# AI4Science-WestlakeU/safediffcon

Measured on AMD Instinct MI355X. Metric: sampled control trajectories/sec (1000-step DDPM), higher is better.
Workload: dtype f32; 1 GPU; C4: 2D smoke Unet3D_with_Conv3D dim=64 (1,2,4) state (B,32,7,64,64), B=64 per GPU, guided 1000-step DDPM, conformal quantile on; batch_per_gpu=64, global_batch=64, step=U-Net + guidance + posterior update of the whole batch, one hipGraph replay, parallelism=batch-sharded x1, no data-path collective, conv_precision=fp32

## Files before the change

### include/sdc.h

```cpp
#ifndef SDC_H
#define SDC_H

#include <stddef.h>
#include <stdint.h>

#ifdef __cplusplus
extern "C" {
#endif

#define SDC_OK 0
#define SDC_EINVAL (-1)
#define SDC_EALIGN (-2)
#define SDC_EHIP (-3)
#define SDC_ENULL (-4)

int sdc_version(void);
int sdc_last_error(char* buf, size_t cap);

typedef struct SdcConvDesc {
    int32_t B, Cin0, Cin1, Cout;
    int32_t iD, iH, iW;
    int32_t oD, oH, oW;
    int32_t kD, kH, kW;
    int32_t sD, sH, sW;
// ... 36 lines not shown

int sdc_chan_norm(const float* x, const float* g, const float* residual, float* y, int B, int C, int64_t S,
                  int mode, float eps, void* stream);

int sdc_linattn(const float* qkv, float* ctx, float* out, int outer, int inner, int heads, int64_t n,
                int64_t q_so, int64_t q_sc, int64_t q_si, int64_t o_so, int64_t o_sc, int64_t o_si, void* stream);

size_t sdc_linattn_block_bytes(int outer, int inner, int C, int64_t n);
int sdc_linattn_block(const float* x, const float* g_pre, const float* wqkv, const float* wo, const float* bo,
                      const float* g_post, float* work, float* y, int outer, int inner, int C, int64_t n,
                      int64_t so, int64_t sc, int64_t si, int pre_mode, int post_mode, float eps, void* stream);
int sdc_linattn_block_gn(const float* x_raw, const float* gn_stats, const float* gn_gamma, const float* gn_beta, int gn_G,
                         const float* gn_residual, const float* g_pre, const float* wqkv, const float* wo, const float* bo,
                         const float* g_post, float* work, float* y, int outer, int inner, int C, int64_t n,
                         int64_t so, int64_t sc, int64_t si, int pre_mode, int post_mode, float eps, void* stream);

size_t sdc_pack_linattn_f16_bytes(int C);
int sdc_pack_linattn_f16(const float* wqkv, const float* wo, int C, void* dst, void* stream);
size_t sdc_linattn_block_f16_bytes(int outer, int inner, int C, int64_t n);
int sdc_linattn_block_f16(const float* x, const float* g_pre, const float* wqkv, const float* wo, const void* wpk, const float* bo,
                          const float* g_post, void* work, float* y, int outer, int inner, int C, int64_t n,
                          int64_t so, int64_t sc, int64_t si, int pre_mode, int post_mode, float eps, void* stream);
int sdc_linattn_block_gn_f16(const float* x_raw, const float* gn_stats, const float* gn_gamma, const float* gn_beta, int gn_G,
                             const float* gn_residual, const float* g_pre, const float* wqkv, const float* wo, const void* wpk,
                             const float* bo, const float* g_post, void* work, float* y, int outer, int inner, int C, int64_t n,
                             int64_t so, int64_t sc, int64_t si, int pre_mode, int post_mode, float eps, void* stream);
int sdc_linattn_block_f16_ok(int C, int64_t n);

int sdc_tattn_block(const float* x, const float* g_pre, const float* wqkv, const float* wo, const float* rot,
                    const float* bias, float* y, int outer, int inner, int C, int ntok, int64_t so, int64_t sc,
// ... 238 lines not shown
```

### safediffcon_amd/_lib.py

```python
import ctypes as C
import os

_HERE = os.path.dirname(os.path.abspath(__file__))
LIB_PATH = os.path.join(_HERE, "libsdc_hip.so")

SDC_MODEL_BURGERS, SDC_MODEL_TOKAMAK, SDC_MODEL_SMOKE = 0, 1, 2

_f32p = C.c_void_p
_i32p = C.c_void_p
_stream = C.c_void_p
_i64 = C.c_int64


class SdcConvDesc(C.Structure):
    _fields_ = [(n, C.c_int32) for n in (
        "B", "Cin0", "Cin1", "Cout", "iD", "iH", "iW", "oD", "oH", "oW", "kD", "kH", "kW", "sD", "sH", "sW",
        "pD", "pH", "pW", "uD", "uH", "uW", "up_mode", "precision")] + [
        ("x0s", C.c_int64 * 5), ("x1s", C.c_int64 * 5), ("ys", C.c_int64 * 5), ("rs", C.c_int64 * 5)]


class SdcStepDesc(C.Structure):
    _fields_ = [(n, C.c_int32) for n in (
        "model", "B", "d0", "d1", "d2", "d3", "guide", "clip", "impose", "cond_idx", "pad_zero", "use_max",
        "has_wgt", "skip_draws", "ddim")] + [("_pad", C.c_int32), ("seed", C.c_uint64)]
# ... 49 lines not shown
    "sdc_gn_apply": (C.c_int, [_f32p, _f32p, _f32p, _f32p, _f32p, _i32p, _i64, _i64, _i64, _f32p, _f32p,
                               C.c_int, C.c_int, C.c_int, _i64, _stream]),
    "sdc_gn_fused_ok": (C.c_int, [C.c_int, C.c_int, C.c_int, _i64]),
    "sdc_gn_fused": (C.c_int, [_f32p, _f32p, _f32p, _f32p, _i32p, _i64, _i64, _i64, _f32p, _f32p, C.c_int, C.c_int, C.c_int, _i64,
                               C.c_float, _stream]),
    "sdc_gn_pointwise_out": (C.c_int, [_f32p, _f32p, _f32p, _f32p, _f32p, _f32p, _f32p, _f32p, C.c_int, C.c_int, C.c_int, C.c_int, _i64,
                                       _i64, _i64, _i64, _i64, _stream]),
    "sdc_chan_norm": (C.c_int, [_f32p, _f32p, _f32p, _f32p, C.c_int, C.c_int, _i64, C.c_int, C.c_float, _stream]),
    "sdc_linattn": (C.c_int, [_f32p, _f32p, _f32p, C.c_int, C.c_int, C.c_int, _i64, _i64, _i64, _i64, _i64, _i64,
                              _i64, _stream]),
    "sdc_linattn_block_bytes": (C.c_size_t, [C.c_int, C.c_int, C.c_int, _i64]),
    "sdc_linattn_block": (C.c_int, [_f32p, _f32p, _f32p, _f32p, _f32p, _f32p, _f32p, _f32p, C.c_int, C.c_int, C.c_int, _i64,
                                    _i64, _i64, _i64, C.c_int, C.c_int, C.c_float, _stream]),
    "sdc_linattn_block_gn": (C.c_int, [_f32p, _f32p, _f32p, _f32p, C.c_int, _f32p, _f32p, _f32p, _f32p, _f32p, _f32p, _f32p, _f32p,
                                       C.c_int, C.c_int, C.c_int, _i64, _i64, _i64, _i64, C.c_int, C.c_int, C.c_float, _stream]),
    "sdc_pack_linattn_f16_bytes": (C.c_size_t, [C.c_int]),
    "sdc_pack_linattn_f16": (C.c_int, [_f32p, _f32p, C.c_int, C.c_void_p, _stream]),
    "sdc_linattn_block_f16_bytes": (C.c_size_t, [C.c_int, C.c_int, C.c_int, _i64]),
    "sdc_linattn_block_f16": (C.c_int, [_f32p, _f32p, _f32p, _f32p, C.c_void_p, _f32p, _f32p, C.c_void_p, _f32p, C.c_int, C.c_int,
                                        C.c_int, _i64, _i64, _i64, _i64, C.c_int, C.c_int, C.c_float, _stream]),
    "sdc_linattn_block_gn_f16": (C.c_int, [_f32p, _f32p, _f32p, _f32p, C.c_int, _f32p, _f32p, _f32p, _f32p, C.c_void_p, _f32p, _f32p,
                                           C.c_void_p, _f32p, C.c_int, C.c_int, C.c_int, _i64, _i64, _i64, _i64, C.c_int, C.c_int,
                                           C.c_float, _stream]),
    "sdc_linattn_block_f16_ok": (C.c_int, [C.c_int, _i64]),
    "sdc_tattn_block": (C.c_int, [_f32p, _f32p, _f32p, _f32p, _f32p, _f32p, _f32p, C.c_int, C.c_int, C.c_int, C.c_int,
                                  _i64, _i64, _i64, C.c_float, _stream]),
    "sdc_pack_tattn_f16_bytes": (C.c_size_t, []),
    "sdc_pack_tattn_f16": (C.c_int, [_f32p, _f32p, C.c_void_p, _stream]),
    "sdc_tattn_block_f16": (C.c_int, [_f32p, _f32p, C.c_void_p, _f32p, _f32p, _f32p, C.c_int, C.c_int, C.c_int, C.c_int,
                                      _i64, _i64, _i64, C.c_float, _stream]),
# ... 124 lines not shown
```

### safediffcon_amd/build.py

```python
import os
import subprocess
import sys

HERE = os.path.dirname(os.path.abspath(__file__))
CSRC = os.path.join(HERE, "csrc")
LIB = os.path.join(HERE, "libsdc_hip.so")
SOURCES = ["sdc_api.hip", "sdc_conv.hip", "sdc_conv_wino.hip", "sdc_conv_f16.hip", "sdc_conv_stem_f16.hip", "sdc_conv_stem_x3.hip", "sdc_conv_gemm_x3.hip", "sdc_conv_wino_x3.hip", "sdc_norm.hip", "sdc_attn.hip", "sdc_lablock.hip", "sdc_lablock_f16.hip", "sdc_tablock.hip", "sdc_tablock_f16.hip", "sdc_tablock_x3.hip", "sdc_step.hip", "sdc_solver.hip", "sdc_grad.hip", "sdc_wgrad_f16.hip", "sdc_attn_bwd.hip", "sdc_kstar.hip", "sdc_smoke.hip", "sdc_linear.hip", "sdc_optim.hip"]
HEADERS = ["sdc_common.h", "sdc_lablock_tile.h", "sdc_conv.h", "sdc_conv_wino3s.inc", "sdc_conv_wino2s.inc", "sdc_conv_pw2.inc"]
HIPCC = os.environ.get("HIPCC", "/opt/rocm/bin/hipcc")
FLAGS = ["--offload-arch=gfx950", "-O3", "-fPIC", "-std=c++17", "-Wall", "-Wno-unused-function"]


def source_hash():
    import hashlib
    h = hashlib.sha256()
    for f in SOURCES + HEADERS:
        with open(os.path.join(CSRC, f), "rb") as fh:
            h.update(fh.read())
    with open(os.path.join(HERE, "..", "include", "sdc.h"), "rb") as fh:
        h.update(fh.read())
    return h.hexdigest()[:16]


def _stale(out, deps):
# ... 44 lines not shown
```

### safediffcon_amd/csrc/sdc_conv_stem_x3.hip

```cpp
#include "sdc_conv.h"

using namespace sdcconv;

namespace {

typedef __bf16 bf16x8 __attribute__((ext_vector_type(8)));

constexpr int SX_BM = 64, SX_BN = 256, SX_NT = 256;

struct StemX3Args {
    const float* x;
    const __bf16* wb;
    const float* bias;
    float* y;
    int64_t xs[5], ys[5];
    int B, Cin, Cout, oD, oH, W, lgW;
    int kD;
    int Hs, NR;
    int Ntot, ntiles, mtiles;
    int itemsB;
    int plane;
};

__device__ __forceinline__ void split3(float x, __bf16& h, __bf16& m, __bf16& l) {
#pragma clang fp contract(off)
    h = (__bf16)x;
    const float r = x - (float)h;
    m = (__bf16)r;
    l = (__bf16)(r - (float)m);
}

template <int KH, int ITB>
__global__ __launch_bounds__(SX_NT) __attribute__((amdgpu_waves_per_eu(1))) SDC_NO_DS_MERGE void conv_stem_x3_kernel(const StemX3Args a) {
    constexpr int TAPS = KH * 7;
    constexpr int NS = (TAPS + 1) / 2;
    constexpr int SS = KH == 7 ? 5 : NS;
    constexpr int NSUB = NS / SS;
    static_assert(NSUB * SS == NS, "whole sub-stages");
    constexpr int HH = KH - 1;
    constexpr int APC = SS * SX_BM * 32;
    constexpr int ASZ = 3 * APC;
    constexpr int NIA = 3 * SS * SX_BM * 2;
    constexpr int ITA = (NIA + SX_NT - 1) / SX_NT;
    extern __shared__ __attribute__((aligned(16))) char lds[];

// ... 267 lines not shown
```

### safediffcon_amd/csrc/sdc_conv_wino_x3.hip

```cpp
#include "sdc_conv.h"

using namespace sdcconv;

namespace {

typedef __bf16 bf16x8 __attribute__((ext_vector_type(8)));
typedef __bf16 bf16x4 __attribute__((ext_vector_type(4)));
typedef float w2f2 __attribute__((ext_vector_type(2)));
typedef float nfloat4 __attribute__((ext_vector_type(4)));
typedef float nfloat2 __attribute__((ext_vector_type(2)));

__device__ __forceinline__ w2f2 pk_add2(w2f2 a, w2f2 b) { w2f2 r; asm("v_pk_add_f32 %0, %1, %2" : "=v"(r) : "v"(a), "v"(b)); return r; }
__device__ __forceinline__ w2f2 pk_sub2(w2f2 a, w2f2 b) { w2f2 r; asm("v_pk_add_f32 %0, %1, %2 neg_lo:[0,1] neg_hi:[0,1]" : "=v"(r) : "v"(a), "v"(b)); return r; }
__device__ __forceinline__ w2f2 pk_fma2(w2f2 a, w2f2 b, w2f2 c) { w2f2 r; asm("v_pk_fma_f32 %0, %1, %2, %3" : "=v"(r) : "v"(a), "v"(b), "v"(c)); return r; }
__device__ __forceinline__ w2f2 pk_fms2(w2f2 a, w2f2 b, w2f2 c) { w2f2 r; asm("v_pk_fma_f32 %0, %1, %2, %3 neg_lo:[0,0,1] neg_hi:[0,0,1]" : "=v"(r) : "v"(a), "v"(b), "v"(c)); return r; }
__device__ __forceinline__ w2f2 pk_fnma2(w2f2 a, w2f2 b, w2f2 c) { w2f2 r; asm("v_pk_fma_f32 %0, %1, %2, %3 neg_lo:[0,1,0] neg_hi:[0,1,0]" : "=v"(r) : "v"(a), "v"(b), "v"(c)); return r; }
__device__ __forceinline__ w2f2 pk_sumdiff(w2f2 c) {
    w2f2 r;
    asm("v_pk_add_f32 %0, %1, %1 op_sel:[0,1] op_sel_hi:[1,0] neg_hi:[0,1]" : "=v"(r) : "v"(c));
    return r;
}
__device__ __forceinline__ w2f2 pk_sumdiff_fwd(w2f2 c) {
    w2f2 r;
    asm("v_pk_add_f32 %0, %1, %1 op_sel:[0,1] op_sel_hi:[0,1] neg_hi:[0,1]" : "=v"(r) : "v"(c));
// ... 22 lines not shown
#pragma unroll
    for (int i = 0; i < 2; ++i) u[i] = (b4 ? w[2 + i] : w[i]) + __shfl_xor(b4 ? w[i] : w[2 + i], 16, 64);
    double t = (b3 ? u[1] : u[0]) + __shfl_xor(b3 ? u[0] : u[1], 8, 64);
    t += __shfl_xor(t, 4, 64);
    t += __shfl_xor(t, 2, 64);
    t += __shfl_xor(t, 1, 64);
    return t;
}

__device__ __forceinline__ uint32_t cvt_pk_bf16(float a, float b) {
    typedef __bf16 bf16x2 __attribute__((ext_vector_type(2)));
    return __builtin_bit_cast(uint32_t, __builtin_convertvector(w2f2{a, b}, bf16x2));
}
__device__ __forceinline__ float bf16_lo(uint32_t p) { return __builtin_bit_cast(float, p << 16); }
__device__ __forceinline__ float bf16_hi(uint32_t p) { return __builtin_bit_cast(float, p & 0xFFFF0000u); }
__device__ __forceinline__ void split3(float x, __bf16& h, __bf16& m, __bf16& l) {
#pragma clang fp contract(off)
    h = (__bf16)x;
    const float r = x - (float)h;
    m = (__bf16)r;
    l = (__bf16)(r - (float)m);
}

constexpr int X3_BM = 64, X3_TILES = 64, X3_SK = 16;
constexpr int X3_PC = 4 * 64 * X3_SK * 2;
constexpr int X3_IMG = 3 * X3_PC;
constexpr int X3_U = 0, X3_V = 2 * X3_IMG;
constexpr int X3_SCR = 4 * X3_IMG;
constexpr int X3_STASH = X3_SCR + 4 * 8 * 8;
constexpr int X3_LDS = X3_STASH + 256 * 8 * 4;
constexpr int X3_RUN = 4 * 64 * X3_SK;

struct WinoX3Args {
    SdcConvDesc d;
    const float* x0;
    const float* x1;
    const __bf16* wb;
// ... 477 lines not shown
```

### safediffcon_amd/csrc/sdc_lablock.hip

```cpp
#include "sdc_common.h"
#include "sdc_lablock_tile.h"

namespace {

struct LaArgs {
    const float* x;
    const float* g_pre;
    const float* wqkv;
    const float* wo;
    const float* bo;
    const float* g_post;
    float* part;
    float* tt;
    float* y;
    const float* gn_stats; const float* gn_gamma; const float* gn_beta; const float* gn_res;
    float* gn_hout;
    int gn_G;
    int inner, nsplit, tiles_per_split, ntiles, tiles_per_blk;
    int pre_mode, post_mode;
    float eps;
    int64_t so, sc, si;
};

template <int C>
__device__ __forceinline__ void norm_tile(float (&v)[C / 4], const float* __restrict__ g, int mode, float eps,
                                          float* __restrict__ xs, float* __restrict__ xr, float* __restrict__ red, int tid) {
    constexpr int CG = C / 4;
    const int tok = tid & 63, grp = tid >> 6;
    if (xr) {
#pragma unroll
        for (int k = 0; k < CG; ++k) xr[(grp * CG + k) * XP + tok] = v[k];
    }
    typedef float la_f2 __attribute__((ext_vector_type(2)));
    la_f2 s2 = {0.f, 0.f};
    if (mode == 0) {
#pragma unroll
        for (int k = 0; k < CG; k += 2) s2 += la_f2{v[k], v[k + 1]};
// ... 355 lines not shown
}

}

extern "C" size_t sdc_linattn_block_bytes(int outer, int inner, int C, int64_t n) {
    if (outer <= 0 || inner <= 0 || n <= 0 || (C != 64 && C != 128)) return 0;
    const int64_t nseq = (int64_t)outer * inner;
    const int ns = pick_nsplit(nseq, (int)(n / TT));
    return sizeof(float) * (size_t)(nseq * ns * 4 * 32 * (C + 2) + nseq * HID * C);
}

namespace {
int linattn_block_impl(const float* x, const float* gn_stats, const float* gn_gamma, const float* gn_beta, int gn_G,
                       const float* gn_res, const float* g_pre, const float* wqkv, const float* wo, const float* bo,
                       const float* g_post, float* work, float* y, int outer, int inner, int C, int64_t n,
                       int64_t so, int64_t sc, int64_t si, int pre_mode, int post_mode, float eps, void* stream) {
    SDC_REQUIRE(x && g_pre && wqkv && wo && work && y, SDC_ENULL, "sdc_linattn_block: null pointer");
    SDC_REQUIRE(C == 64 || C == 128, SDC_EINVAL, "sdc_linattn_block: dim must be 64 or 128 (got %d)", C);
    SDC_REQUIRE(outer > 0 && inner > 0 && n > 0 && n % TT == 0, SDC_EINVAL, "sdc_linattn_block: tokens must be a multiple of 64");
    SDC_REQUIRE((pre_mode == 0 || pre_mode == 1) && post_mode >= -1 && post_mode <= 1, SDC_EINVAL, "sdc_linattn_block: bad norm mode");
    SDC_REQUIRE(post_mode < 0 || g_post, SDC_ENULL, "sdc_linattn_block: post norm needs its gain");
    const int64_t nseq = (int64_t)outer * inner;
    SDC_REQUIRE(nseq < 65536, SDC_EINVAL, "sdc_linattn_block: outer*inner must be < 65536");
    SDC_REQUIRE(sc > 0 && sc < (1ll << 27), SDC_EINVAL, "sdc_linattn_block: channel stride must stay below 2^27 elements (32-bit lane offsets)");
    LaArgs a;
    a.x = x; a.g_pre = g_pre; a.wqkv = wqkv; a.wo = wo; a.bo = bo; a.g_post = g_post; a.y = y;
    a.gn_stats = gn_stats; a.gn_gamma = gn_gamma; a.gn_beta = gn_beta; a.gn_res = gn_res; a.gn_G = gn_G; a.gn_hout = nullptr;
    a.inner = inner; a.ntiles = (int)(n / TT);
    a.nsplit = pick_nsplit(nseq, a.ntiles);
    a.tiles_per_split = (a.ntiles + a.nsplit - 1) / a.nsplit;
    a.nsplit = (a.ntiles + a.tiles_per_split - 1) / a.tiles_per_split;
    {
// ... 7 lines not shown
    a.so = so; a.sc = sc; a.si = si;
    hipStream_t s = sdc::as_stream(stream);
    const dim3 g1((unsigned)a.nsplit, (unsigned)nseq), gm(4, (unsigned)nseq),
        g2((unsigned)((a.ntiles + a.tiles_per_blk - 1) / a.tiles_per_blk), (unsigned)nseq);
    const size_t ldsb = sizeof(float) * (size_t)((C + HID) * XP + 8 * TT + 2 * C);
    const size_t ldsb2 = sizeof(float) * (size_t)((C + HID) * XP + 8 * TT + C * XP + 2 * C);
    static std::atomic<uint64_t> attr0{0}, attr1{0}, attr2{0};
    static std::atomic<uint64_t> attr3{0};
    SDC_LDS_OPTIN(attr0, (la_blk_ctx<128, false>), 96 * 1024, "sdc_linattn_block");
    SDC_LDS_OPTIN(attr1, la_blk_out<128>, 128 * 1024, "sdc_linattn_block");
    SDC_LDS_OPTIN(attr2, la_blk_out<64>, 96 * 1024, "sdc_linattn_block");
    SDC_LDS_OPTIN(attr3, (la_blk_ctx<128, true>), 96 * 1024, "sdc_linattn_block");
    const bool gn = gn_stats != nullptr;
    LaArgs a2 = a;
    if (gn) { a.gn_hout = y; a2.x = y; a2.gn_stats = nullptr; }
    if (C == 64) {
        if (gn) hipLaunchKernelGGL((la_blk_ctx<64, true>), g1, dim3(NT), ldsb, s, a);
        else hipLaunchKernelGGL((la_blk_ctx<64, false>), g1, dim3(NT), ldsb, s, a);
        hipLaunchKernelGGL(la_blk_mid<64>, gm, dim3(NT), 0, s, a);
        hipLaunchKernelGGL(la_blk_out<64>, g2, dim3(NT), ldsb2, s, a2);
    } else {
        if (gn) hipLaunchKernelGGL((la_blk_ctx<128, true>), g1, dim3(NT), ldsb, s, a);
        else hipLaunchKernelGGL((la_blk_ctx<128, false>), g1, dim3(NT), ldsb, s, a);
        hipLaunchKernelGGL(la_blk_mid<128>, gm, dim3(NT), 0, s, a);
        hipLaunchKernelGGL(la_blk_out<128>, g2, dim3(NT), ldsb2, s, a2);
    }
    return sdc::check_launch("sdc_linattn_block");
}
}

extern "C" int sdc_linattn_block(const float* x, const float* g_pre, const float* wqkv, const float* wo, const float* bo,
                                 const float* g_post, float* work, float* y, int outer, int inner, int C, int64_t n,
                                 int64_t so, int64_t sc, int64_t si, int pre_mode, int post_mode, float eps, void* stream) {
    return linattn_block_impl(x, nullptr, nullptr, nullptr, 0, nullptr, g_pre, wqkv, wo, bo, g_post, work, y, outer, inner, C, n, so, sc,
                              si, pre_mode, post_mode, eps, stream);
}

extern "C" int sdc_linattn_block_gn(const float* x_raw, const float* gn_stats, const float* gn_gamma, const float* gn_beta, int gn_G,
                                    const float* gn_residual, const float* g_pre, const float* wqkv, const float* wo, const float* bo,
                                    const float* g_post, float* work, float* y, int outer, int inner, int C, int64_t n,
                                    int64_t so, int64_t sc, int64_t si, int pre_mode, int post_mode, float eps, void* stream) {
    SDC_REQUIRE(gn_stats && gn_gamma && gn_beta, SDC_ENULL, "sdc_linattn_block_gn: null GroupNorm pointer");
    SDC_REQUIRE(gn_G > 0 && (C == 64 || C == 128) && C % gn_G == 0, SDC_EINVAL, "sdc_linattn_block_gn: groups must divide the channels");
    return linattn_block_impl(x_raw, gn_stats, gn_gamma, gn_beta, gn_G, gn_residual, g_pre, wqkv, wo, bo, g_post, work, y, outer, inner,
                              C, n, so, sc, si, pre_mode, post_mode, eps, stream);
}
```

### safediffcon_amd/csrc/sdc_lablock_tile.h

```cpp
#pragma once
#include "sdc_common.h"

namespace {

constexpr int NT = 256;
constexpr int TT = 64;
constexpr int XP = TT + 1;
constexpr int HID = 128;
constexpr float LOG2E = 1.4426950408889634f;
typedef float f32x16 __attribute__((ext_vector_type(16)));

typedef __attribute__((address_space(1))) float* la_gptr;
typedef __attribute__((address_space(1))) char* la_gcptr;
__device__ __forceinline__ la_gptr la_uni(const float* p) {
    const uint64_t u = reinterpret_cast<uint64_t>(p);
    const uint32_t lo = __builtin_amdgcn_readfirstlane((uint32_t)u), hi = __builtin_amdgcn_readfirstlane((uint32_t)(u >> 32));
    return (la_gptr)(((uint64_t)hi << 32) | lo);
}
__device__ __forceinline__ float la_ld(la_gptr base, uint32_t byte_off) { return *(la_gptr)((la_gcptr)base + byte_off); }
__device__ __forceinline__ void la_st(la_gptr base, uint32_t byte_off, float v) { *(la_gptr)((la_gcptr)base + byte_off) = v; }

__device__ __forceinline__ float la_max3(float a, float b, float c) { float r; asm("v_max3_f32 %0, %1, %2, %3" : "=v"(r) : "v"(a), "v"(b), "v"(c)); return r; }

template <int C>
// ... 60 lines not shown
```

### safediffcon_amd/csrc/sdc_tablock_x3.hip

```cpp
#include "sdc_common.h"

namespace {

constexpr int NT = 512;
constexpr int C = 64;
constexpr int NS = 8;
constexpr int XP = NS * 33;
constexpr int XF = 68;
constexpr int XPP = 32 * XF + 8;
constexpr int WQKV_E = 3 * 4 * 64 * 8;
constexpr int HEAD_E = WQKV_E + 2 * 2 * 64 * 8;
constexpr int WPK_E = 4 * 3 * HEAD_E;
constexpr int WBUF_B = 3 * HEAD_E * 2;
constexpr int REGB_B = NS * XPP * 4;
typedef float f32x16 __attribute__((ext_vector_type(16)));
typedef float nfloat4 __attribute__((ext_vector_type(4)));
typedef __bf16 bf16x8 __attribute__((ext_vector_type(8)));
typedef uint32_t u32x4 __attribute__((ext_vector_type(4)));
static_assert(WBUF_B <= REGB_B && 32 * XP * 4 <= REGB_B, "region B holds a head's weights and a y half");
static_assert(WBUF_B % (16 * NT) == 0, "whole 16-byte words per thread");

struct TaArgs {
    const float* x; const float* g; const __bf16* wpk; const float* rot; const float* bias;
    float* y;
// ... 8 lines not shown
typedef __attribute__((address_space(1))) float* gptr_t;
typedef __attribute__((address_space(1))) char* gcptr_t;
__device__ __forceinline__ gptr_t uni(const float* p) {
    const uint64_t u = reinterpret_cast<uint64_t>(p);
    const uint32_t lo = __builtin_amdgcn_readfirstlane((uint32_t)u), hi = __builtin_amdgcn_readfirstlane((uint32_t)(u >> 32));
    return (gptr_t)(((uint64_t)hi << 32) | lo);
}
__device__ __forceinline__ float ldu(gptr_t base, uint32_t byte_off) { return *(gptr_t)((gcptr_t)base + byte_off); }
__device__ __forceinline__ void stu(gptr_t base, uint32_t byte_off, float v) { *(gptr_t)((gcptr_t)base + byte_off) = v; }

typedef float ta2 __attribute__((ext_vector_type(2)));
__device__ __forceinline__ ta2 ta_rot(ta2 x, ta2 cs) {
#pragma clang fp contract(off)
    const float t0 = x.x * cs.x, t1 = x.y * cs.x;
    return ta2{__builtin_fmaf(-x.y, cs.y, t0), __builtin_fmaf(x.x, cs.y, t1)};
}

__device__ __forceinline__ void split3(float x, __bf16& h, __bf16& m, __bf16& l) {
#pragma clang fp contract(off)
    h = (__bf16)x;
    const float r = x - (float)h;
    m = (__bf16)r;
    l = (__bf16)(r - (float)m);
}

__global__ __launch_bounds__(NT) void ta_block_x3_kernel(const TaArgs a) {
    extern __shared__ __attribute__((aligned(16))) unsigned char smem_x3[];
    unsigned char* const wA = smem_x3;
    unsigned char* const rB = smem_x3 + WBUF_B;
    float* const xim = reinterpret_cast<float*>(rB);
    float* const ys = reinterpret_cast<float*>(rB);
    float* const biasT = reinterpret_cast<float*>(rB + REGB_B);
    float* const rotcs = biasT + 4 * 32 * 33;
    float* const red = rotcs + 2 * 32 * 16;

    const int tid = threadIdx.x, lane = tid & 63, wave = tid >> 6, l31 = lane & 31, lh = lane >> 5;
    const int nblk = a.nblk, nwg = gridDim.x, w = blockIdx.x;
    const bool xcd = ((nblk & 7) == 0) && ((nwg & 7) == 0);
// ... 258 lines not shown
```

Baseline: 0.3024 trajectories/s.

## Add bf16x3 split MFMA path for linear-attention block context and output kernels

Adds new context and output kernels for the linear-attention block. Activations and weights are split into three bf16 pieces so the projections run on bf16 MFMA while keeping accuracy close to fp32, and the default entry points now take this path for supported channel and token counts. The split3 helper moves into a shared header and the LaArgs struct is exposed so the new kernels can use it. The cost is the split work and larger LDS use per block, which may limit how many blocks fit on a CU.

Measured after the change: 0.3068 trajectories/s, median of 6. +1.5%, better.

```diff
diff --git a/include/sdc.h b/include/sdc.h
--- a/include/sdc.h
+++ b/include/sdc.h
@@ -74,6 +74,14 @@
                          const float* gn_residual, const float* g_pre, const float* wqkv, const float* wo, const float* bo,
                          const float* g_post, float* work, float* y, int outer, int inner, int C, int64_t n,
                          int64_t so, int64_t sc, int64_t si, int pre_mode, int post_mode, float eps, void* stream);
+int sdc_linattn_block_sel(const float* x, const float* g_pre, const float* wqkv, const float* wo, const float* bo,
+                          const float* g_post, float* work, float* y, int outer, int inner, int C, int64_t n,
+                          int64_t so, int64_t sc, int64_t si, int pre_mode, int post_mode, float eps, int impl, void* stream);
+int sdc_linattn_block_gn_sel(const float* x_raw, const float* gn_stats, const float* gn_gamma, const float* gn_beta, int gn_G,
+                             const float* gn_residual, const float* g_pre, const float* wqkv, const float* wo, const float* bo,
+                             const float* g_post, float* work, float* y, int outer, int inner, int C, int64_t n,
+                             int64_t so, int64_t sc, int64_t si, int pre_mode, int post_mode, float eps, int impl, void* stream);
+int sdc_linattn_block_x3_ok(int C, int64_t n);
 
 size_t sdc_pack_linattn_f16_bytes(int C);
 int sdc_pack_linattn_f16(const float* wqkv, const float* wo, int C, void* dst, void* stream);
diff --git a/safediffcon_amd/_lib.py b/safediffcon_amd/_lib.py
--- a/safediffcon_amd/_lib.py
+++ b/safediffcon_amd/_lib.py
@@ -87,6 +87,11 @@
                                     _i64, _i64, _i64, C.c_int, C.c_int, C.c_float, _stream]),
     "sdc_linattn_block_gn": (C.c_int, [_f32p, _f32p, _f32p, _f32p, C.c_int, _f32p, _f32p, _f32p, _f32p, _f32p, _f32p, _f32p, _f32p,
                                        C.c_int, C.c_int, C.c_int, _i64, _i64, _i64, _i64, C.c_int, C.c_int, C.c_float, _stream]),
+    "sdc_linattn_block_sel": (C.c_int, [_f32p, _f32p, _f32p, _f32p, _f32p, _f32p, _f32p, _f32p, C.c_int, C.c_int, C.c_int, _i64,
+                                        _i64, _i64, _i64, C.c_int, C.c_int, C.c_float, C.c_int, _stream]),
+    "sdc_linattn_block_gn_sel": (C.c_int, [_f32p, _f32p, _f32p, _f32p, C.c_int, _f32p, _f32p, _f32p, _f32p, _f32p, _f32p, _f32p, _f32p,
+                                           C.c_int, C.c_int, C.c_int, _i64, _i64, _i64, _i64, C.c_int, C.c_int, C.c_float, C.c_int, _stream]),
+    "sdc_linattn_block_x3_ok": (C.c_int, [C.c_int, _i64]),
     "sdc_pack_linattn_f16_bytes": (C.c_size_t, [C.c_int]),
     "sdc_pack_linattn_f16": (C.c_int, [_f32p, _f32p, C.c_int, C.c_void_p, _stream]),
     "sdc_linattn_block_f16_bytes": (C.c_size_t, [C.c_int, C.c_int, C.c_int, _i64]),
diff --git a/safediffcon_amd/build.py b/safediffcon_amd/build.py
--- a/safediffcon_amd/build.py
+++ b/safediffcon_amd/build.py
@@ -5,8 +5,8 @@
 HERE = os.path.dirname(os.path.abspath(__file__))
 CSRC = os.path.join(HERE, "csrc")
 LIB = os.path.join(HERE, "libsdc_hip.so")
-SOURCES = ["sdc_api.hip", "sdc_conv.hip", "sdc_conv_wino.hip", "sdc_conv_f16.hip", "sdc_conv_stem_f16.hip", "sdc_conv_stem_x3.hip", "sdc_conv_gemm_x3.hip", "sdc_conv_wino_x3.hip", "sdc_norm.hip", "sdc_attn.hip", "sdc_lablock.hip", "sdc_lablock_f16.hip", "sdc_tablock.hip", "sdc_tablock_f16.hip", "sdc_tablock_x3.hip", "sdc_step.hip", "sdc_solver.hip", "sdc_grad.hip", "sdc_wgrad_f16.hip", "sdc_attn_bwd.hip", "sdc_kstar.hip", "sdc_smoke.hip", "sdc_linear.hip", "sdc_optim.hip"]
-HEADERS = ["sdc_common.h", "sdc_lablock_tile.h", "sdc_conv.h", "sdc_conv_wino3s.inc", "sdc_conv_wino2s.inc", "sdc_conv_pw2.inc"]
+SOURCES = ["sdc_api.hip", "sdc_conv.hip", "sdc_conv_wino.hip", "sdc_conv_f16.hip", "sdc_conv_stem_f16.hip", "sdc_conv_stem_x3.hip", "sdc_conv_gemm_x3.hip", "sdc_conv_wino_x3.hip", "sdc_norm.hip", "sdc_attn.hip", "sdc_lablock.hip", "sdc_lablock_f16.hip", "sdc_lablock_x3.hip", "sdc_tablock.hip", "sdc_tablock_f16.hip", "sdc_tablock_x3.hip", "sdc_step.hip", "sdc_solver.hip", "sdc_grad.hip", "sdc_wgrad_f16.hip", "sdc_attn_bwd.hip", "sdc_kstar.hip", "sdc_smoke.hip", "sdc_linear.hip", "sdc_optim.hip"]
+HEADERS = ["sdc_common.h", "sdc_lablock_tile.h", "sdc_split3.h", "sdc_conv.h", "sdc_conv_wino3s.inc", "sdc_conv_wino2s.inc", "sdc_conv_pw2.inc"]
 HIPCC = os.environ.get("HIPCC", "/opt/rocm/bin/hipcc")
 FLAGS = ["--offload-arch=gfx950", "-O3", "-fPIC", "-std=c++17", "-Wall", "-Wno-unused-function"]
 
diff --git a/safediffcon_amd/csrc/sdc_conv_stem_x3.hip b/safediffcon_amd/csrc/sdc_conv_stem_x3.hip
--- a/safediffcon_amd/csrc/sdc_conv_stem_x3.hip
+++ b/safediffcon_amd/csrc/sdc_conv_stem_x3.hip
@@ -1,4 +1,5 @@
 #include "sdc_conv.h"
+#include "sdc_split3.h"
 
 using namespace sdcconv;
 
@@ -21,14 +22,6 @@
     int itemsB;
     int plane;
 };
-
-__device__ __forceinline__ void split3(float x, __bf16& h, __bf16& m, __bf16& l) {
-#pragma clang fp contract(off)
-    h = (__bf16)x;
-    const float r = x - (float)h;
-    m = (__bf16)r;
-    l = (__bf16)(r - (float)m);
-}
 
 template <int KH, int ITB>
 __global__ __launch_bounds__(SX_NT) __attribute__((amdgpu_waves_per_eu(1))) SDC_NO_DS_MERGE void conv_stem_x3_kernel(const StemX3Args a) {
diff --git a/safediffcon_amd/csrc/sdc_conv_wino_x3.hip b/safediffcon_amd/csrc/sdc_conv_wino_x3.hip
--- a/safediffcon_amd/csrc/sdc_conv_wino_x3.hip
+++ b/safediffcon_amd/csrc/sdc_conv_wino_x3.hip
@@ -1,4 +1,5 @@
 #include "sdc_conv.h"
+#include "sdc_split3.h"
 
 using namespace sdcconv;
 
@@ -60,13 +61,6 @@
 }
 __device__ __forceinline__ float bf16_lo(uint32_t p) { return __builtin_bit_cast(float, p << 16); }
 __device__ __forceinline__ float bf16_hi(uint32_t p) { return __builtin_bit_cast(float, p & 0xFFFF0000u); }
-__device__ __forceinline__ void split3(float x, __bf16& h, __bf16& m, __bf16& l) {
-#pragma clang fp contract(off)
-    h = (__bf16)x;
-    const float r = x - (float)h;
-    m = (__bf16)r;
-    l = (__bf16)(r - (float)m);
-}
 
 constexpr int X3_BM = 64, X3_TILES = 64, X3_SK = 16;
 constexpr int X3_PC = 4 * 64 * X3_SK * 2;
diff --git a/safediffcon_amd/csrc/sdc_lablock.hip b/safediffcon_amd/csrc/sdc_lablock.hip
--- a/safediffcon_amd/csrc/sdc_lablock.hip
+++ b/safediffcon_amd/csrc/sdc_lablock.hip
@@ -2,25 +2,6 @@
 #include "sdc_lablock_tile.h"
 
 namespace {
-
-struct LaArgs {
-    const float* x;
-    const float* g_pre;
-    const float* wqkv;
-    const float* wo;
-    const float* bo;
-    const float* g_post;
-    float* part;
-    float* tt;
-    float* y;
-    const float* gn_stats; const float* gn_gamma; const float* gn_beta; const float* gn_res;
-    float* gn_hout;
-    int gn_G;
-    int inner, nsplit, tiles_per_split, ntiles, tiles_per_blk;
-    int pre_mode, post_mode;
-    float eps;
-    int64_t so, sc, si;
-};
 
 template <int C>
 __device__ __forceinline__ void norm_tile(float (&v)[C / 4], const float* __restrict__ g, int mode, float eps,
@@ -406,8 +387,9 @@
 int linattn_block_impl(const float* x, const float* gn_stats, const float* gn_gamma, const float* gn_beta, int gn_G,
                        const float* gn_res, const float* g_pre, const float* wqkv, const float* wo, const float* bo,
                        const float* g_post, float* work, float* y, int outer, int inner, int C, int64_t n,
-                       int64_t so, int64_t sc, int64_t si, int pre_mode, int post_mode, float eps, void* stream) {
+                       int64_t so, int64_t sc, int64_t si, int pre_mode, int post_mode, float eps, int impl, void* stream) {
     SDC_REQUIRE(x && g_pre && wqkv && wo && work && y, SDC_ENULL, "sdc_linattn_block: null pointer");
+    SDC_REQUIRE(impl == 0 || impl == 1, SDC_EINVAL, "sdc_linattn_block: impl must be 0 or 1 (got %d)", impl);
     SDC_REQUIRE(C == 64 || C == 128, SDC_EINVAL, "sdc_linattn_block: dim must be 64 or 128 (got %d)", C);
     SDC_REQUIRE(outer > 0 && inner > 0 && n > 0 && n % TT == 0, SDC_EINVAL, "sdc_linattn_block: tokens must be a multiple of 64");
     SDC_REQUIRE((pre_mode == 0 || pre_mode == 1) && post_mode >= -1 && post_mode <= 1, SDC_EINVAL, "sdc_linattn_block: bad norm mode");
@@ -445,7 +427,14 @@
     const bool gn = gn_stats != nullptr;
     LaArgs a2 = a;
     if (gn) { a.gn_hout = y; a2.x = y; a2.gn_stats = nullptr; }
-    if (C == 64) {
+    if (impl == 1) {
+        int rc = sdc::la_x3_launch_ctx(a, C, gn, g1, s);
+        if (rc != SDC_OK) return rc;
+        if (C == 64) hipLaunchKernelGGL(la_blk_mid<64>, gm, dim3(NT), 0, s, a);
+        else hipLaunchKernelGGL(la_blk_mid<128>, gm, dim3(NT), 0, s, a);
+        rc = sdc::la_x3_launch_out(a2, C, g2, s);
+        if (rc != SDC_OK) return rc;
+    } else if (C == 64) {
         if (gn) hipLaunchKernelGGL((la_blk_ctx<64, true>), g1, dim3(NT), ldsb, s, a);
         else hipLaunchKernelGGL((la_blk_ctx<64, false>), g1, dim3(NT), ldsb, s, a);
         hipLaunchKernelGGL(la_blk_mid<64>, gm, dim3(NT), 0, s, a);
@@ -460,19 +449,34 @@
 }
 }
 
+extern "C" int sdc_linattn_block_sel(const float* x, const float* g_pre, const float* wqkv, const float* wo, const float* bo,
+                                     const float* g_post, float* work, float* y, int outer, int inner, int C, int64_t n,
+                                     int64_t so, int64_t sc, int64_t si, int pre_mode, int post_mode, float eps, int impl, void* stream) {
+    return linattn_block_impl(x, nullptr, nullptr, nullptr, 0, nullptr, g_pre, wqkv, wo, bo, g_post, work, y, outer, inner, C, n, so, sc,
+                              si, pre_mode, post_mode, eps, impl, stream);
+}
+
 extern "C" int sdc_linattn_block(const float* x, const float* g_pre, const float* wqkv, const float* wo, const float* bo,
                                  const float* g_post, float* work, float* y, int outer, int inner, int C, int64_t n,
                                  int64_t so, int64_t sc, int64_t si, int pre_mode, int post_mode, float eps, void* stream) {
-    return linattn_block_impl(x, nullptr, nullptr, nullptr, 0, nullptr, g_pre, wqkv, wo, bo, g_post, work, y, outer, inner, C, n, so, sc,
-                              si, pre_mode, post_mode, eps, stream);
+    return sdc_linattn_block_sel(x, g_pre, wqkv, wo, bo, g_post, work, y, outer, inner, C, n, so, sc, si, pre_mode, post_mode, eps,
+                                 sdc_linattn_block_x3_ok(C, n), stream);
+}
+
+extern "C" int sdc_linattn_block_gn_sel(const float* x_raw, const float* gn_stats, const float* gn_gamma, const float* gn_beta, int gn_G,
+                                        const float* gn_residual, const float* g_pre, const float* wqkv, const float* wo, const float* bo,
+                                        const float* g_post, float* work, float* y, int outer, int inner, int C, int64_t n,
+                                        int64_t so, int64_t sc, int64_t si, int pre_mode, int post_mode, float eps, int impl, void* stream) {
+    SDC_REQUIRE(gn_stats && gn_gamma && gn_beta, SDC_ENULL, "sdc_linattn_block_gn: null GroupNorm pointer");
+    SDC_REQUIRE(gn_G > 0 && (C == 64 || C == 128) && C % gn_G == 0, SDC_EINVAL, "sdc_linattn_block_gn: groups must divide the channels");
+    return linattn_block_impl(x_raw, gn_stats, gn_gamma, gn_beta, gn_G, gn_residual, g_pre, wqkv, wo, bo, g_post, work, y, outer, inner,
+                              C, n, so, sc, si, pre_mode, post_mode, eps, impl, stream);
 }
 
 extern "C" int sdc_linattn_block_gn(const float* x_raw, const float* gn_stats, const float* gn_gamma, const float* gn_beta, int gn_G,
                                     const float* gn_residual, const float* g_pre, const float* wqkv, const float* wo, const float* bo,
                                     const float* g_post, float* work, float* y, int outer, int inner, int C, int64_t n,
                                     int64_t so, int64_t sc, int64_t si, int pre_mode, int post_mode, float eps, void* stream) {
-    SDC_REQUIRE(gn_stats && gn_gamma && gn_beta, SDC_ENULL, "sdc_linattn_block_gn: null GroupNorm pointer");
-    SDC_REQUIRE(gn_G > 0 && (C == 64 || C == 128) && C % gn_G == 0, SDC_EINVAL, "sdc_linattn_block_gn: groups must divide the channels");
-    return linattn_block_impl(x_raw, gn_stats, gn_gamma, gn_beta, gn_G, gn_residual, g_pre, wqkv, wo, bo, g_post, work, y, outer, inner,
-                              C, n, so, sc, si, pre_mode, post_mode, eps, stream);
-}
+    return sdc_linattn_block_gn_sel(x_raw, gn_stats, gn_gamma, gn_beta, gn_G, gn_residual, g_pre, wqkv, wo, bo, g_post, work, y, outer,
+                                    inner, C, n, so, sc, si, pre_mode, post_mode, eps, sdc_linattn_block_x3_ok(C, n), stream);
+}
diff --git a/safediffcon_amd/csrc/sdc_lablock_tile.h b/safediffcon_amd/csrc/sdc_lablock_tile.h
--- a/safediffcon_amd/csrc/sdc_lablock_tile.h
+++ b/safediffcon_amd/csrc/sdc_lablock_tile.h
@@ -1,7 +1,35 @@
 #pragma once
 #include "sdc_common.h"
 
+namespace sdc {
+
+struct LaArgs {
+    const float* x;
+    const float* g_pre;
+    const float* wqkv;
+    const float* wo;
+    const float* bo;
+    const float* g_post;
+    float* part;
+    float* tt;
+    float* y;
+    const float* gn_stats; const float* gn_gamma; const float* gn_beta; const float* gn_res;
+    float* gn_hout;
+    int gn_G;
+    int inner, nsplit, tiles_per_split, ntiles, tiles_per_blk;
+    int pre_mode, post_mode;
+    float eps;
+    int64_t so, sc, si;
+};
+
+int la_x3_launch_ctx(const LaArgs& a, int C, bool gn, dim3 grid, hipStream_t stream);
+int la_x3_launch_out(const LaArgs& a, int C, dim3 grid, hipStream_t stream);
+
+}
+
 namespace {
+
+using sdc::LaArgs;
 
 constexpr int NT = 256;
 constexpr int TT = 64;
diff --git a/safediffcon_amd/csrc/sdc_lablock_x3.hip b/safediffcon_amd/csrc/sdc_lablock_x3.hip
--- /dev/null
+++ b/safediffcon_amd/csrc/sdc_lablock_x3.hip
@@ -0,0 +1,413 @@
+#include "sdc_common.h"
+#include "sdc_lablock_tile.h"
+#include "sdc_split3.h"
+
+namespace {
+
+typedef __bf16 bf16x8 __attribute__((ext_vector_type(8)));
+__host__ __device__ constexpr int cpitch(int C) { return C + 8; }
+constexpr int PRE_CTX64 = 3, PRE_OUT64 = 1;
+__device__ __forceinline__ float x3_max3(float a, float b, float c) { return fmaxf(fmaxf(a, b), c); }
+__host__ __device__ constexpr int piece_e(int C) { return TT * cpitch(C); }
+
+template <int C>
+__device__ __forceinline__ void norm_tile_x3(float (&v)[C / 4], const float* __restrict__ g, int mode, float eps, float* __restrict__ xs,
+                                             __bf16* __restrict__ xt, float* __restrict__ xr, float* __restrict__ red, int tid) {
+    constexpr int CG = C / 4, CP = cpitch(C);
+    const int tok = tid & 63, grp = tid >> 6;
+    if (xr) {
+#pragma unroll
+        for (int k = 0; k < CG; ++k) xr[(grp * CG + k) * XP + tok] = v[k];
+    }
+    typedef float la_f2 __attribute__((ext_vector_type(2)));
+    la_f2 s2 = {0.f, 0.f};
+    float o[CG];
+    if (mode == 0) {
+#pragma unroll
+        for (int k = 0; k < CG; k += 2) s2 += la_f2{v[k], v[k + 1]};
+        red[grp * TT + tok] = s2.x + s2.y;
+        __syncthreads();
+        const float mean = (red[tok] + red[TT + tok] + red[2 * TT + tok] + red[3 * TT + tok]) * (1.0f / C);
+        const la_f2 m2 = {mean, mean};
+        la_f2 q2 = {0.f, 0.f};
+#pragma unroll
+        for (int k = 0; k < CG; k += 2) {
+            const la_f2 d2 = la_f2{v[k], v[k + 1]} - m2;
+            v[k] = d2.x; v[k + 1] = d2.y;
+            q2 += d2 * d2;
+        }
+        red[(4 + grp) * TT + tok] = q2.x + q2.y;
+        __syncthreads();
+        const float var = (red[4 * TT + tok] + red[5 * TT + tok] + red[6 * TT + tok] + red[7 * TT + tok]) * (1.0f / C);
+        const float rstd = rsqrtf(var + eps);
+        const la_f2 r2 = {rstd, rstd};
+#pragma unroll
+        for (int k = 0; k < CG; k += 2) {
+            const la_f2 o2 = la_f2{v[k], v[k + 1]} * r2 * la_f2{g[grp * CG + k], g[grp * CG + k + 1]};
+            o[k] = o2.x; o[k + 1] = o2.y;
+        }
+    } else {
+#pragma unroll
+        for (int k = 0; k < CG; k += 2) { const la_f2 d2 = {v[k], v[k + 1]}; s2 += d2 * d2; }
+        red[grp * TT + tok] = s2.x + s2.y;
+        __syncthreads();
+        const float nrm = sqrtf(red[tok] + red[TT + tok] + red[2 * TT + tok] + red[3 * TT + tok]);
+        const float f = sqrtf((float)C) / fmaxf(nrm, 1e-12f);
+        const la_f2 f2 = {f, f};
+#pragma unroll
+        for (int k = 0; k < CG; k += 2) {
+            const la_f2 o2 = la_f2{v[k], v[k + 1]} * f2 * la_f2{g[grp * CG + k], g[grp * CG + k + 1]};
+            o[k] = o2.x; o[k + 1] = o2.y;
+        }
+    }
+    if (xs) {
+#pragma unroll
+        for (int k = 0; k < CG; ++k) xs[(grp * CG + k) * XP + tok] = o[k];
+    }
+    bf16x8* xo = reinterpret_cast<bf16x8*>(xt + tok * CP + grp * CG);
+#pragma unroll
+    for (int c8 = 0; c8 < CG / 8; ++c8) {
+        bf16x8 ph, pm, pl;
+#pragma unroll
+        for (int j = 0; j < 8; ++j) {
+            __bf16 h, m, l;
+            split3(o[c8 * 8 + j], h, m, l);
+            ph[j] = h; pm[j] = m; pl[j] = l;
+        }
+        xo[c8] = ph;
+        xo[piece_e(C) / 8 + c8] = pm;
+        xo[2 * (piece_e(C) / 8) + c8] = pl;
+    }
+    __syncthreads();
+}
+
+template <int C>
+__device__ __forceinline__ void split_weight(const float* __restrict__ wqkv, int col, int lh, bf16x8 (&w)[3][C / 16]) {
+#pragma unroll
+    for (int s = 0; s < C / 16; ++s)
+#pragma unroll
+        for (int j = 0; j < 8; ++j) {
+            __bf16 h, m, l;
+            split3(wqkv[(int64_t)(16 * s + 8 * lh + j) * (3 * HID) + col], h, m, l);
+            w[0][s][j] = h; w[1][s][j] = m; w[2][s][j] = l;
+        }
+}
+
+template <int C, bool XA, int NPRE>
+__device__ __forceinline__ void project_x3(const bf16x8 (&w)[3][C / 16], const __bf16* __restrict__ xt, int l31, int lh, f32x16 (&acc)[2]) {
+    constexpr int NKS = C / 16, CP8 = cpitch(C) / 8, PE8 = piece_e(C) / 8;
+    constexpr int PA[6] = {2, 1, 0, 1, 0, 0}, PB[6] = {0, 1, 2, 0, 1, 0};
+#pragma unroll
+    for (int r = 0; r < 16; ++r) { acc[0][r] = 0.f; acc[1][r] = 0.f; }
+    const bf16x8* xp = reinterpret_cast<const bf16x8*>(xt) + l31 * CP8 + lh;
+    bf16x8 xf[NPRE > 0 ? NPRE : 1][2][NKS];
+#pragma unroll
+    for (int p = 0; p < NPRE; ++p)
+#pragma unroll
+        for (int j = 0; j < 2; ++j)
+#pragma unroll
+            for (int s = 0; s < NKS; ++s) xf[p][j][s] = xp[p * PE8 + j * 32 * CP8 + 2 * s];
+#pragma unroll
+    for (int t = 0; t < 6; ++t) {
+#pragma unroll
+        for (int s = 0; s < NKS; ++s)
+#pragma unroll
+            for (int j = 0; j < 2; ++j) {
+                const bf16x8 xv = PB[t] < NPRE ? xf[PB[t] < NPRE ? PB[t] : 0][j][s] : xp[PB[t] * PE8 + j * 32 * CP8 + 2 * s];
+                acc[j] = XA ? __builtin_amdgcn_mfma_f32_32x32x16_bf16(xv, w[PA[t]][s], acc[j], 0, 0, 0)
+                            : __builtin_amdgcn_mfma_f32_32x32x16_bf16(w[PA[t]][s], xv, acc[j], 0, 0, 0);
+            }
+        if (C == 64 && NPRE < 3) __builtin_amdgcn_sched_barrier(0);
+    }
+}
+
+template <int C, bool GN>
+__global__ __launch_bounds__(NT, (C == 64 ? 2 : 1)) SDC_NO_DS_MERGE void la_x3_ctx(const LaArgs a) {
+    constexpr int NCT = C / 32;
+    extern __shared__ __attribute__((aligned(16))) unsigned char smem_x3[];
+    __bf16* const xt = reinterpret_cast<__bf16*>(smem_x3);
+    float* const xs = reinterpret_cast<float*>(xt + 3 * piece_e(C));
+    float* const red = xs + C * XP;
+    float* const gcoef = red + 8 * TT;
+    const int tid = threadIdx.x, lane = tid & 63, head = tid >> 6, l31 = lane & 31, lh = lane >> 5;
+    const int split = blockIdx.x, seq = blockIdx.y;
+    const int o = seq / a.inner, i = seq - o * a.inner;
+    const float* xseq = a.x + o * a.so + i * a.si;
+    const float* rseq = (GN && a.gn_res) ? a.gn_res + o * a.so + i * a.si : nullptr;
+    if (GN) gn_coef_fill<C>(a.gn_stats, a.gn_gamma, a.gn_beta, a.gn_G, o, gcoef, tid);
+
+    bf16x8 wk[3][C / 16];
+    split_weight<C>(a.wqkv, HID + head * 32 + l31, lh, wk);
+
+    f32x16 macc[NCT];
+#pragma unroll
+    for (int t = 0; t < NCT; ++t)
+#pragma unroll
+        for (int r = 0; r < 16; ++r) macc[t][r] = 0.f;
+    float mrun = -INFINITY, psum = 0.f;
+
+    const int t0 = split * a.tiles_per_split;
+    const int t1 = min(t0 + a.tiles_per_split, a.ntiles);
+    float xv[C / 4];
+    if (t0 < t1) fetch_tile<C>(xseq + (int64_t)t0 * TT, a.sc, tid, xv);
+    if (GN) __syncthreads();
+    for (int tile = t0; tile < t1; ++tile) {
+        if (GN) {
+            gn_apply_tile<C>(xv, rseq ? rseq + (int64_t)tile * TT : nullptr, a.sc, gcoef, tid);
+            float* hb = a.gn_hout + o * a.so + i * a.si + (int64_t)tile * TT;
+            constexpr int CG = C / 4;
+            la_gptr hp = la_uni(hb + (int64_t)(__builtin_amdgcn_readfirstlane(tid >> 6) * CG) * a.sc);
+            uint32_t hoff = (uint32_t)(tid & 63) * 4u;
+#pragma unroll
+            for (int k = 0; k < CG; ++k) {
+                asm volatile("" : "+v"(hoff));
+                la_st(hp, hoff, xv[k]);
+                hp += a.sc;
+                asm volatile("" : "+s"(hp));
+            }
+        }
+        norm_tile_x3<C>(xv, a.g_pre, a.pre_mode, a.eps, xs, xt, nullptr, red, tid);
+        if (tile + 1 < t1) fetch_tile<C>(xseq + (int64_t)(tile + 1) * TT, a.sc, tid, xv);
+        f32x16 kacc[2];
+        project_x3<C, true, (C == 64 ? PRE_CTX64 : 0)>(wk, xt, l31, lh, kacc);
+        float tmax = kacc[0][0];
+#pragma unroll
+        for (int r = 0; r < 16; ++r) tmax = x3_max3(tmax, kacc[0][r], kacc[1][r]);
+        tmax = fmaxf(tmax, __shfl_xor(tmax, 32, 64));
+        const float mnew = fmaxf(mrun, tmax);
+        const float f = __expf(mrun - mnew);
+        mrun = mnew;
+        float ps = 0.f;
+        const float nml = -mnew * LOG2E;
+#pragma unroll
+        for (int r = 0; r < 16; ++r) {
+            kacc[0][r] = __builtin_amdgcn_exp2f(fmaf(kacc[0][r], LOG2E, nml));
+            kacc[1][r] = __builtin_amdgcn_exp2f(fmaf(kacc[1][r], LOG2E, nml));
+            ps += kacc[0][r] + kacc[1][r];
+        }
+        psum = psum * f + ps;
+        if (__builtin_amdgcn_ballot_w64(f != 1.0f)) {
+#pragma unroll
+            for (int t = 0; t < NCT; ++t)
+#pragma unroll
+                for (int r = 0; r < 16; ++r) macc[t][r] *= f;
+        }
+#pragma unroll
+        for (int j = 0; j < 2; ++j)
+#pragma unroll
+            for (int r = 0; r < 16; ++r) {
+                const int tok = j * 32 + (r & 3) + 8 * (r >> 2) + 4 * lh;
+#pragma unroll
+                for (int t = 0; t < NCT; ++t)
+                    macc[t] = __builtin_amdgcn_mfma_f32_32x32x2f32(xs[(t * 32 + l31) * XP + tok], kacc[j][r], macc[t], 0, 0, 0);
+            }
+        __syncthreads();
+    }
+    float* pp = a.part + (((int64_t)seq * a.nsplit + split) * 4 + head) * (32 * (C + 2));
+#pragma unroll
+    for (int t = 0; t < NCT; ++t)
+#pragma unroll
+        for (int r = 0; r < 16; ++r) pp[l31 * C + t * 32 + (r & 3) + 8 * (r >> 2) + 4 * lh] = macc[t][r];
+    const float stot = psum + __shfl_xor(psum, 32, 64);
+    if (lh == 0) { pp[32 * C + l31] = mrun; pp[32 * C + 32 + l31] = stot; }
+}
+
+template <int C>
+__global__ __launch_bounds__(NT, (C == 64 ? 2 : 1)) SDC_NO_DS_MERGE void la_x3_out(const LaArgs a) {
+    constexpr int NRT = C / 32;
+    constexpr int TPW = NRT / 2;
+    extern __shared__ __attribute__((aligned(16))) unsigned char smem_x3[];
+    __bf16* const xt = reinterpret_cast<__bf16*>(smem_x3);
+    float* const qs = reinterpret_cast<float*>(xt + 3 * piece_e(C));
+    float* const red = qs + HID * XP;
+    float* const xr = red + 8 * TT;
+    float* const bg = xr + C * XP;
+    const int tid = threadIdx.x, lane = tid & 63, wave = tid >> 6, l31 = lane & 31, lh = lane >> 5;
+    const int seq = blockIdx.y;
+    const int o = seq / a.inner, i = seq - o * a.inner;
+    const float* xseq = a.x + o * a.so + i * a.si;
+    float* yseq = a.y + o * a.so + i * a.si;
+    const int rt = (NRT == 2) ? (wave & 1) : wave;
+    const int ct0 = (NRT == 2) ? (wave >> 1) : 0;
+
+    bf16x8 wq[3][C / 16];
+    split_weight<C>(a.wqkv, wave * 32 + l31, lh, wq);
+    float treg[HID / 2];
+    const float* tb = a.tt + (int64_t)seq * HID * C;
+#pragma unroll
+    for (int ks = 0; ks < HID / 2; ++ks) treg[ks] = tb[(2 * ks + lh) * C + rt * 32 + l31];
+    for (int c = tid; c < C; c += NT) {
+        bg[c] = a.bo ? a.bo[c] : 0.f;
+        bg[C + c] = a.g_post ? a.g_post[c] : 1.f;
+    }
+
+    const int t0 = blockIdx.x * a.tiles_per_blk;
+    const int t1 = min(t0 + a.tiles_per_blk, a.ntiles);
+    float xv[C / 4];
+    if (t0 < t1) fetch_tile<C>(xseq + (int64_t)t0 * TT, a.sc, tid, xv);
+    for (int tile = t0; tile < t1; ++tile) {
+        norm_tile_x3<C>(xv, a.g_pre, a.pre_mode, a.eps, nullptr, xt, xr, red, tid);
+        if (tile + 1 < t1) fetch_tile<C>(xseq + (int64_t)(tile + 1) * TT, a.sc, tid, xv);
+        f32x16 qacc[2];
+        project_x3<C, false, (C == 64 ? PRE_OUT64 : 0)>(wq, xt, l31, lh, qacc);
+#pragma unroll
+        for (int j = 0; j < 2; ++j) {
+            float m = fmaxf(qacc[j][0], qacc[j][1]);
+#pragma unroll
+            for (int r = 2; r < 16; r += 2) m = x3_max3(m, qacc[j][r], qacc[j][r + 1]);
+            m = fmaxf(m, __shfl_xor(m, 32, 64));
+            typedef float la_f2 __attribute__((ext_vector_type(2)));
+            const float nml = -m * LOG2E;
+            const la_f2 l2 = {LOG2E, LOG2E}, n2 = {nml, nml};
+            la_f2 s2 = {0.f, 0.f};
+#pragma unroll
+            for (int r = 0; r < 16; r += 2) {
+                const la_f2 e2 = la_f2{qacc[j][r], qacc[j][r + 1]} * l2 + n2;
+                const la_f2 p2 = {__builtin_amdgcn_exp2f(e2.x), __builtin_amdgcn_exp2f(e2.y)};
+                qacc[j][r] = p2.x; qacc[j][r + 1] = p2.y;
+                s2 += p2;
+            }
+            float s = s2.x + s2.y;
+            s += __shfl_xor(s, 32, 64);
+            const float f = 0.17677669529663687f * __builtin_amdgcn_rcpf(s);
+            const la_f2 f2 = {f, f};
+#pragma unroll
+            for (int r = 0; r < 16; r += 2) {
+                const la_f2 o2 = la_f2{qacc[j][r], qacc[j][r + 1]} * f2;
+                qs[(wave * 32 + (r & 3) + 8 * (r >> 2) + 4 * lh) * XP + j * 32 + l31] = o2.x;
+                qs[(wave * 32 + ((r + 1) & 3) + 8 * ((r + 1) >> 2) + 4 * lh) * XP + j * 32 + l31] = o2.y;
+            }
+        }
+        __syncthreads();
+        f32x16 yacc[TPW];
+#pragma unroll
+        for (int u = 0; u < TPW; ++u)
+#pragma unroll
+            for (int r = 0; r < 16; ++r) yacc[u][r] = bg[rt * 32 + (r & 3) + 8 * (r >> 2) + 4 * lh];
+#pragma unroll
+        for (int ks = 0; ks < HID / 2; ++ks)
+#pragma unroll
+            for (int u = 0; u < TPW; ++u)
+                yacc[u] = __builtin_amdgcn_mfma_f32_32x32x2f32(treg[ks], qs[(2 * ks + lh) * XP + (ct0 + u) * 32 + l31], yacc[u], 0, 0, 0);
+        if (a.post_mode >= 0) {
+            float st[TPW];
+#pragma unroll
+            for (int u = 0; u < TPW; ++u) {
+                float s = 0.f;
+                if (a.post_mode == 0) {
+#pragma unroll
+                    for (int r = 0; r < 16; ++r) s += yacc[u][r];
+                } else {
+#pragma unroll
+                    for (int r = 0; r < 16; ++r) s += yacc[u][r] * yacc[u][r];
+                }
+                s += __shfl_xor(s, 32, 64);
+                if (lh == 0) red[rt * TT + (ct0 + u) * 32 + l31] = s;
+            }
+            __syncthreads();
+#pragma unroll
+            for (int u = 0; u < TPW; ++u) {
+                float s = 0.f;
+#pragma unroll
+                for (int q = 0; q < NRT; ++q) s += red[q * TT + (ct0 + u) * 32 + l31];
+                st[u] = s;
+            }
+            if (a.post_mode == 0) {
+#pragma unroll
+                for (int u = 0; u < TPW; ++u) {
+                    typedef float la_f2 __attribute__((ext_vector_type(2)));
+                    const float mean = st[u] * (1.0f / C);
+                    const la_f2 m2 = {mean, mean};
+                    la_f2 q2 = {0.f, 0.f};
+#pragma unroll
+                    for (int r = 0; r < 16; r += 2) {
+                        const la_f2 d2 = la_f2{yacc[u][r], yacc[u][r + 1]} - m2;
+                        yacc[u][r] = d2.x; yacc[u][r + 1] = d2.y;
+                        q2 += d2 * d2;
+                    }
+                    float q = q2.x + q2.y;
+                    q += __shfl_xor(q, 32, 64);
+                    if (lh == 0) red[(4 + rt) * TT + (ct0 + u) * 32 + l31] = q;
+                }
+                __syncthreads();
+#pragma unroll
+                for (int u = 0; u < TPW; ++u) {
+                    float q = 0.f;
+#pragma unroll
+                    for (int w = 0; w < NRT; ++w) q += red[(4 + w) * TT + (ct0 + u) * 32 + l31];
+                    const float rstd = rsqrtf(q * (1.0f / C) + a.eps);
+                    typedef float la_f2 __attribute__((ext_vector_type(2)));
+                    const la_f2 r2 = {rstd, rstd};
+#pragma unroll
+                    for (int r = 0; r < 16; r += 2) {
+                        const la_f2 o2 = la_f2{yacc[u][r], yacc[u][r + 1]} * r2 *
+                                         la_f2{bg[C + rt * 32 + (r & 3) + 8 * (r >> 2) + 4 * lh], bg[C + rt * 32 + ((r + 1) & 3) + 8 * ((r + 1) >> 2) + 4 * lh]};
+                        yacc[u][r] = o2.x; yacc[u][r + 1] = o2.y;
+                    }
+                }
+            } else {
+#pragma unroll
+                for (int u = 0; u < TPW; ++u) {
+                    const float f = sqrtf((float)C) / fmaxf(sqrtf(st[u]), 1e-12f);
+#pragma unroll
+                    for (int r = 0; r < 16; ++r) yacc[u][r] = yacc[u][r] * f * bg[C + rt * 32 + (r & 3) + 8 * (r >> 2) + 4 * lh];
+                }
+            }
+        }
+#pragma unroll
+        for (int u = 0; u < TPW; ++u) {
+            const int col = (ct0 + u) * 32 + l31;
+            uint32_t loff = (uint32_t)((int64_t)(4 * lh) * a.sc + col) * 4u;
+            la_gptr yrow = la_uni(yseq + (int64_t)(rt * 32) * a.sc + (int64_t)tile * TT);
+            const float* xrow = xr + (rt * 32 + 4 * lh) * XP + col;
+#pragma unroll
+            for (int r = 0; r < 16; ++r) {
+                asm volatile("" : "+v"(loff));
+                la_st(yrow, loff, yacc[u][r] + xrow[((r & 3) + 8 * (r >> 2)) * XP]);
+                yrow += ((r & 3) == 3 ? 5 : 1) * a.sc;
+                asm volatile("" : "+s"(yrow));
+            }
+        }
+        __syncthreads();
+    }
+}
+
+size_t lds_ctx(int C) { return sizeof(__bf16) * (size_t)(3 * piece_e(C)) + sizeof(float) * (size_t)(C * XP + 8 * TT + 2 * C); }
+size_t lds_out(int C) { return sizeof(__bf16) * (size_t)(3 * piece_e(C)) + sizeof(float) * (size_t)(HID * XP + 8 * TT + C * XP + 2 * C); }
+static_assert((sizeof(__bf16) * 3 * piece_e(64)) % 16 == 0 && (sizeof(__bf16) * 3 * piece_e(128)) % 16 == 0, "the fp32 images start on 16 bytes");
+static_assert(2 * (sizeof(__bf16) * 3 * piece_e(64) + sizeof(float) * (HID * XP + 8 * TT + 64 * XP + 2 * 64)) <= 160 * 1024, "la_x3_out<64>: two per CU");
+
+}
+
+namespace sdc {
+
+int la_x3_launch_ctx(const LaArgs& a, int C, bool gn, dim3 grid, hipStream_t stream) {
+    static std::atomic<uint64_t> attr0{0}, attr1{0};
+    SDC_LDS_OPTIN(attr0, (la_x3_ctx<128, false>), 96 * 1024, "sdc_linattn_block");
+    SDC_LDS_OPTIN(attr1, (la_x3_ctx<128, true>), 96 * 1024, "sdc_linattn_block");
+    const size_t ldsb = lds_ctx(C);
+    if (C == 64) {
+        if (gn) hipLaunchKernelGGL((la_x3_ctx<64, true>), grid, dim3(NT), ldsb, stream, a);
+        else hipLaunchKernelGGL((la_x3_ctx<64, false>), grid, dim3(NT), ldsb, stream, a);
+    } else {
+        if (gn) hipLaunchKernelGGL((la_x3_ctx<128, true>), grid, dim3(NT), ldsb, stream, a);
+        else hipLaunchKernelGGL((la_x3_ctx<128, false>), grid, dim3(NT), ldsb, stream, a);
+    }
+    return SDC_OK;
+}
+
+int la_x3_launch_out(const LaArgs& a, int C, dim3 grid, hipStream_t stream) {
+    static std::atomic<uint64_t> attr0{0}, attr1{0};
+    SDC_LDS_OPTIN(attr0, la_x3_out<64>, 96 * 1024, "sdc_linattn_block");
+    SDC_LDS_OPTIN(attr1, la_x3_out<128>, 128 * 1024, "sdc_linattn_block");
+    const size_t ldsb = lds_out(C);
+    if (C == 64) hipLaunchKernelGGL(la_x3_out<64>, grid, dim3(NT), ldsb, stream, a);
+    else hipLaunchKernelGGL(la_x3_out<128>, grid, dim3(NT), ldsb, stream, a);
+    return SDC_OK;
+}
+
+}
+
+extern "C" int sdc_linattn_block_x3_ok(int C, int64_t n) {
+    return (C == 64 && (n == 4096 || n == 2048 || n == 1024)) || (C == 128 && (n == 1024 || n == 512));
+}
diff --git a/safediffcon_amd/csrc/sdc_split3.h b/safediffcon_amd/csrc/sdc_split3.h
--- /dev/null
+++ b/safediffcon_amd/csrc/sdc_split3.h
@@ -0,0 +1,14 @@
+#pragma once
+#include "sdc_common.h"
+
+namespace {
+
+__device__ __forceinline__ void split3(float x, __bf16& h, __bf16& m, __bf16& l) {
+#pragma clang fp contract(off)
+    h = (__bf16)x;
+    const float r = x - (float)h;
+    m = (__bf16)r;
+    l = (__bf16)(r - (float)m);
+}
+
+}
diff --git a/safediffcon_amd/csrc/sdc_tablock_x3.hip b/safediffcon_amd/csrc/sdc_tablock_x3.hip
--- a/safediffcon_amd/csrc/sdc_tablock_x3.hip
+++ b/safediffcon_amd/csrc/sdc_tablock_x3.hip
@@ -1,4 +1,5 @@
 #include "sdc_common.h"
+#include "sdc_split3.h"
 
 namespace {
 
@@ -46,14 +47,6 @@
 #pragma clang fp contract(off)
     const float t0 = x.x * cs.x, t1 = x.y * cs.x;
     return ta2{__builtin_fmaf(-x.y, cs.y, t0), __builtin_fmaf(x.x, cs.y, t1)};
-}
-
-__device__ __forceinline__ void split3(float x, __bf16& h, __bf16& m, __bf16& l) {
-#pragma clang fp contract(off)
-    h = (__bf16)x;
-    const float r = x - (float)h;
-    m = (__bf16)r;
-    l = (__bf16)(r - (float)m);
 }
 
 __global__ __launch_bounds__(NT) void ta_block_x3_kernel(const TaArgs a) {
```
